# facebookresearch/momentum

Measured on NVIDIA H100. Metric: GN iterations/sec (batched 72-joint IK), higher is better.
Workload: dtype f32

## Files before the change

include/momentum_b200.h:

```cpp
#ifndef MOMENTUM_B200_H_
#define MOMENTUM_B200_H_

#include <stddef.h>
#include <stdint.h>

#ifdef __cplusplus
extern "C" {
#endif

#define MB2_PARAMETERS_PER_JOINT 7
#define MB2_MAX_MODEL_PARAMETERS 2048
#define MB2_PARAMETER_SET_WORDS 32

typedef enum mb2_status {
  MB2_OK = 0,
  MB2_ERR_INVALID_ARGUMENT = 1,
  MB2_ERR_CUDA = 2,
  MB2_ERR_UNSUPPORTED = 3
} mb2_status;

typedef enum mb2_instance_status {
  MB2_INSTANCE_OK = 0,
  MB2_INSTANCE_CHOLESKY_BREAKDOWN = 1,
  MB2_INSTANCE_NON_FINITE = 2
// ... 152 lines not shown
int mb2_solver_create(mb2_solver_function* f, const mb2_gauss_newton_options* opt, mb2_solver** out);
void mb2_solver_destroy(mb2_solver* s);
int mb2_solver_set_options(mb2_solver* s, const mb2_gauss_newton_options* opt);
int mb2_solver_set_enabled_parameters(mb2_solver* s, const uint64_t bits[MB2_PARAMETER_SET_WORDS]);
int mb2_solver_solve(mb2_solver* s, float* parameters, double* errors, int32_t* iterations, int32_t* status);
int mb2_solver_solve_async(mb2_solver* s, float* parameters);
int mb2_solver_wait(mb2_solver* s, double* errors, int32_t* iterations, int32_t* status);
int mb2_solver_solve_device(mb2_solver* s, float* parameters_device, void* cuda_stream);
int mb2_solver_get_results(mb2_solver* s, double* errors, int32_t* iterations, int32_t* status);
int mb2_solver_get_error_history(mb2_solver* s, double* history);
int mb2_solver_get_counters(mb2_solver* s, uint64_t* total_iterations, uint64_t* kernel_launches);
int mb2_solver_set_profiling(mb2_solver* s, int32_t enabled);
int mb2_solver_get_phase_times(mb2_solver* s, double ms[4], uint64_t launches[4]);
int mb2_solver_get_plan_stats(mb2_solver* s, int64_t stats[12]);
int mb2_solver_get_fused_profile(mb2_solver* s, int32_t* fused, int32_t* groups, double* kernel_ms, uint64_t phase_cycles[12]);
int mb2_solver_function_get_sweep_launch(mb2_solver_function* f, int32_t jacobian, int64_t out[5]);
int mb2_solver_get_solve_path(mb2_solver* s, int64_t out[15]);

typedef struct mb2_mixed_batch mb2_mixed_batch;
const char* mb2_mixed_batch_last_error(void);
int mb2_mixed_batch_create(int device, int32_t granule , mb2_mixed_batch** out);
void mb2_mixed_batch_destroy(mb2_mixed_batch* b);
int mb2_mixed_batch_add_rig(mb2_mixed_batch* b, const mb2_character* c, int32_t num_parameters, int32_t* rig_id);
int mb2_mixed_batch_use_limits(mb2_mixed_batch* b, int32_t enabled, float weight);
int mb2_mixed_batch_add_instance(mb2_mixed_batch* b, int32_t rig_id, int32_t num_constraints, const int32_t* parents, const float* offsets ,
                                 const float* weights , const float* targets , const float* theta0 , int32_t* instance_id);
int mb2_mixed_batch_set_parameters(mb2_mixed_batch* b, int32_t instance_id, const float* theta0);
int mb2_mixed_batch_solve(mb2_mixed_batch* b, const mb2_gauss_newton_options* opt);
int mb2_mixed_batch_get_result(mb2_mixed_batch* b, int32_t instance_id, float* theta, double* error, int32_t* iterations, int32_t* status);
int mb2_mixed_batch_get_results(mb2_mixed_batch* b, float* theta, const int64_t* theta_offsets, double* errors, int32_t* iterations, int32_t* status);
// ... 27 lines not shown
```

momentum_b200/csrc/ik_capi.cu:

```cuda
#include "../../include/momentum_b200.h"

#include <cuda_runtime.h>
#include <nvtx3/nvToolsExt.h>

#include <algorithm>
#include <cfloat>
#include <cmath>
#include <cstdio>
#include <cstdlib>
#include <cstring>
#include <memory>
#include <string>
#include <vector>

#include "ik_chol_sched.h"
#include "ik_fused.cuh"
#include "ik_jtj_tc.cuh"
#include "ik_kernels.cuh"
#include "ik_plan.h"
#include "ik_solve_path.h"

using namespace mb2;

namespace {
// ... 105 lines not shown
  const mb2_character* ch{nullptr};
  int B{0};
  cudaStream_t stream{nullptr};
  HostFunction host;
  bool planDirty{true};
  int planMode{0};
  bool planSchedDense{false};
  bool planAlignRows{false};
  uint64_t planLimitsVersion{~0ull};
  Plan plan;
  int ldJ{32};
  DeviceBuffer<EfDesc> dEfs;
  DeviceBuffer<UnitDesc> dUnits;
  DeviceBuffer<CellDesc> dCells;
  DeviceBuffer<ContribDesc> dContribs;
  DeviceBuffer<float> dLimitData;
  DeviceBuffer<int32_t> dEnabledList, dIdentity, dDeviceCols;
  DeviceBuffer<float> dTargets, dWeights, dJ, dTheta, dState, dH, dTargetStage;
  DeviceBuffer<double> dErrors;
  DeviceBuffer<double> dJacobi;
  std::unique_ptr<DeviceSchedule> sched;
  SweepLaunch lastSweep[2]{};
  FunctionTables tables() const;
};

struct PhaseEvent {
  cudaEvent_t start, stop;
  int phase;
};

struct mb2_solver {
  mb2_solver_function* fn{nullptr};
  mb2_gauss_newton_options opt{};
  DeviceBuffer<float> dH, dDelta, dThetaOrig, dTheta0, dScale, dGradDotDelta, dThetaStage, dGrad, dTiles, dRadius, dRSaved;
  DeviceBuffer<double> dLastErrors, dTrialErrors, dHistory;
  DeviceBuffer<int32_t> dActive, dIterations, dStatus, dSearching, dActiveCount, dWorkCounter, dQrChunks;
  DeviceBuffer<unsigned long long> dPhaseCycles;
  DeviceBuffer<float> dPark;
  DeviceBuffer<uint32_t> dParkSlots;
  SolvePath path;
  cudaEvent_t fusedStart{nullptr}, fusedStop{nullptr};
  double fusedMs{0};
  int* hActiveCount{nullptr};
  char* hResults{nullptr};
  size_t hResultsBytes{0};
  bool resultsStaged{false};
  uint64_t totalIterations{0}, kernelLaunches{0};
  bool profiling{false};
  bool inKernelProfile{false};
  std::vector<PhaseEvent> events;
  double phaseMs[4]{0, 0, 0, 0};
  uint64_t phaseLaunches[4]{0, 0, 0, 0};
// ... 36 lines not shown
  T.contribs = dContribs.p;
  T.limitData = dLimitData.p;
  T.targetStride = host.targetStride;
  T.recStride = plan.recStride;
  T.numRows = plan.numRows;
  T.ldJ = ldJ;
  T.numCols = plan.numCols;
  T.weightsPerInstance = host.weightsPerInstance ? 1 : 0;
  T.numWeights = host.numWeights;
  T.numContribs = int(plan.contribs.size());
  T.numLimitData = int(plan.limitData.size());
  const bool strips = planMode == 2 && planAlignRows && sched;
  T.stripMode = strips ? 1 : 0;
  T.residOff = strips ? sched->gram.residOff : 0;
  T.jacobianStride = strips ? size_t(sched->gram.stride) : size_t(plan.numCols + 1) * ldJ;
  return T;
}

namespace {

bool g_deviceChecked = false;
int g_usableDevices = 0;
}
namespace {
int usableDevices() {
  if (!g_deviceChecked) {
    int n = 0;
    if (cudaGetDeviceCount(&n) != cudaSuccess) { n = 0; cudaGetLastError(); }
    int ok = 0;
    for (int d = 0; d < n; ++d) {
// ... 72 lines not shown
        std::copy(ds->gc.tab.begin(), ds->gc.tab.end(), ds->gcParams->tab);
      } else if (ds->gcValid) {
        MB2_CUDA(ds->gcTab.upload(ds->gc.tab, s));
      }
      MB2_CUDA(ds->fBlob.upload(makeFusedBlob(f->ch->host, f->plan, gblob, sblob, ds->fLayout), s));
    }
    f->sched = std::move(ds);
  }
  f->planMode = mode;
  f->planSchedDense = schedDense;
  f->planAlignRows = alignRows;
  MB2_CUDA(f->dEfs.upload(f->plan.efs, s));
  MB2_CUDA(f->dUnits.upload(f->plan.units, s));
  MB2_CUDA(f->dCells.upload(f->plan.cells, s));
  MB2_CUDA(f->dContribs.upload(f->plan.contribs, s));
  MB2_CUDA(f->dLimitData.upload(f->plan.limitData, s));
  MB2_CUDA(f->dEnabledList.upload(f->plan.enabledList, s));
  MB2_CUDA(f->dDeviceCols.upload(f->plan.deviceCols, s));
  std::vector<int32_t> ident(f->ch->host.numParams);
  for (size_t i = 0; i < ident.size(); ++i) ident[i] = int32_t(i);
  MB2_CUDA(f->dIdentity.upload(ident, s));
  f->ldJ = std::max(32, roundUp(f->plan.numRows, 32));
  const bool stripLayout = mode == 2 && alignRows;
  const size_t jElems = stripLayout ? size_t(f->B) * size_t(f->sched->gram.stride) : size_t(f->B) * (f->plan.numCols + 1) * f->ldJ;
  MB2_CUDA(f->dJ.resize(jElems));
  MB2_CUDA(cudaMemsetAsync(f->dJ.p, 0, jElems * sizeof(float), s));
  MB2_CUDA(f->dErrors.resize(f->B));
  MB2_CUDA(f->dTheta.resize(size_t(f->B) * f->ch->host.numParams));
  int rc = ensureTargets(f);
  if (rc != MB2_OK) return rc;
// ... 846 lines not shown
  MB2_CUDA(s->dDelta.resize(size_t(B) * ns));
  MB2_CUDA(s->dTheta0.resize(size_t(B) * n));
  MB2_CUDA(s->dLastErrors.resize(B));
  MB2_CUDA(s->dActive.resize(B));
  MB2_CUDA(s->dActiveCount.resize(1));
  const bool lineSearch = o.do_line_search != 0 && P.kind != kSolveTrustRegionQr;
  if (lineSearch) {
    MB2_CUDA(s->dThetaOrig.resize(size_t(B) * n));
    MB2_CUDA(s->dTrialErrors.resize(B));
    MB2_CUDA(s->dScale.resize(B));
    MB2_CUDA(s->dSearching.resize(B));
    MB2_CUDA(s->dGradDotDelta.resize(B));
  }
  double* history = o.store_error_history ? s->dHistory.p : nullptr;

  const SweepArgs sweep = sweepArgs(f, theta, s->dActive.p);
  GramArgs g{};
  if (P.strips) {
    const DeviceSchedule& ds = *f->sched;
    g.batch = B;
    g.strips = f->dJ.p;
    g.stripStride = size_t(ds.gram.stride);
    g.residOff = ds.gram.residOff;
    g.active = s->dActive.p;
    g.numStrips = ds.gram.numStrips;
    g.numTiles = ds.host.numTiles;
    g.numTileCols = ds.host.numTileCols;
    g.nPad = ds.host.nPad;
    g.numOrder = int32_t(ds.gram.tileOrder.size());
    g.blob = ds.gBlob.p;
    g.blobInts = ds.gBlobInts;
// ... 287 lines not shown
    if ((persistent || gramChol) && s->profiling && s->dPhaseCycles.p) {
      MB2_DEVICE_GUARD(s->fn->ch->device);
      unsigned long long h[12];
      MB2_CUDA(cudaMemcpy(h, s->dPhaseCycles.p, sizeof(h), cudaMemcpyDeviceToHost));
      if (persistent) {
        for (int k = 0; k < 12; ++k) phaseCycles[k] = h[k];
      } else {
        phaseCycles[0] = h[0];
        for (int k = 1; k < 8; ++k) phaseCycles[4 + k] = h[k];
      }
    }
  }
  return MB2_OK;
}

int mb2_solver_function_get_sweep_launch(mb2_solver_function* f, int32_t jacobian, int64_t out[5]) {
  MB2_CHECK(f != nullptr && out != nullptr, "null argument");
  const SweepLaunch& l = f->lastSweep[jacobian ? 1 : 0];
  out[0] = l.stageTables;
  out[1] = l.warpsPerInstance;
  out[2] = l.groupsPerCta;
  out[3] = l.grid;
  out[4] = l.smemBytes;
  return MB2_OK;
}

int mb2_solver_get_solve_path(mb2_solver* s, int64_t out[15]) {
  MB2_CHECK(s != nullptr && out != nullptr, "null argument");
  solvePathWords(s->path, out);
  return MB2_OK;
// ... 13 lines not shown
```

momentum_b200/csrc/ik_device.cuh:

```cuda
#pragma once

#include <cmath>
#include <cfloat>

#include "ik_types.h"

namespace mb2 {

struct F3 {
  float x, y, z;
};
struct Q4 {
  float x, y, z, w;
};

MB2_HD F3 f3(float x, float y, float z) { F3 r; r.x = x; r.y = y; r.z = z; return r; }
MB2_HD F3 operator+(F3 a, F3 b) { return f3(a.x + b.x, a.y + b.y, a.z + b.z); }
MB2_HD F3 operator-(F3 a, F3 b) { return f3(a.x - b.x, a.y - b.y, a.z - b.z); }
MB2_HD F3 operator*(F3 a, float s) { return f3(a.x * s, a.y * s, a.z * s); }
MB2_HD F3 operator*(float s, F3 a) { return f3(a.x * s, a.y * s, a.z * s); }
MB2_HD float dot(F3 a, F3 b) { return a.x * b.x + a.y * b.y + a.z * b.z; }
MB2_HD F3 cross(F3 a, F3 b) { return f3(a.y * b.z - a.z * b.y, a.z * b.x - a.x * b.z, a.x * b.y - a.y * b.x); }
MB2_HD float comp(F3 a, int i) { return i == 0 ? a.x : (i == 1 ? a.y : a.z); }

// ... 260 lines not shown
#endif
  }
};
template <int kThreads>
struct CtaLanes {
  static constexpr int size = kThreads;
  int lane;
  MB2_HD void sync() const {
#if defined(__CUDA_ARCH__)
    __syncthreads();
#endif
  }
};
#endif

template <bool kAxes, bool kFromJointParameters, class Lanes>
MB2_HD void fkPasses(const Lanes& g, const CharacterTables& C, const float* src, float* js) {
  for (int j = g.lane; j < C.numJoints; j += g.size) {
    if constexpr (kFromJointParameters) fkLocal<kAxes>(C, j, src, js);
    else fkLocalFromTheta<kAxes>(C, j, src, js);
  }
  g.sync();
  for (int lvl = 1; lvl < C.numLevels; ++lvl) {
    const int end = C.levelStart[lvl + 1];
    for (int k = C.levelStart[lvl] + g.lane; k < end; k += g.size) fkCompose(C, C.levelJoints[k], js);
    g.sync();
  }
  if constexpr (kAxes)
    for (int i = g.lane; i < 3 * C.numJoints; i += g.size) fkAxis(C, i / 3, i % 3, js);
}

template <class Lanes>
MB2_HD void skelGradPasses(const Lanes& g, const CharacterTables& C, const SkeletonTables& S, const float* js, const float* grad, float* acc,
                           float* gjp, float* out) {
  for (int i = g.lane; i < C.numJoints; i += g.size) skelGradSeed(js, i, grad + 8 * i, acc);
  g.sync();
  for (int lvl = C.numLevels - 2; lvl >= 0; --lvl) {
    const int end = C.levelStart[lvl + 1];
    for (int k = C.levelStart[lvl] + g.lane; k < end; k += g.size) skelGradFold(S, js, C.levelJoints[k], acc);
    g.sync();
  }
  for (int row = g.lane; row < C.numJoints * kParametersPerJoint; row += g.size) gjp[row] = skelGradJointParameter(C, js, acc, row);
// ... 463 lines not shown
            }
          }
        }
      }
      const int nr = lm ? 6 : 12;
      for (int k = 0; k < nr; ++k) out[MB2_ROW(k)] = acc[k];
      break;
    }
    default:
      out[MB2_ROW(0)] = rc[0] * c.coef;
      break;
  }
#undef MB2_ROW
}

MB2_HD void skinTransform(const float* state, const float* ibp, float* m) {
  const Q4 q = qnormalized(ld4(state + 3));
  const float s = state[7];
  float R[9];
  qmat(q, R);
  for (int r = 0; r < 3; ++r) {
    const F3 sr = f3(s * R[r], s * R[3 + r], s * R[6 + r]);
    m[4 * r + 0] = dot(sr, f3(ibp[0], ibp[4], ibp[8]));
    m[4 * r + 1] = dot(sr, f3(ibp[1], ibp[5], ibp[9]));
    m[4 * r + 2] = dot(sr, f3(ibp[2], ibp[6], ibp[10]));
    m[4 * r + 3] = dot(sr, f3(ibp[3], ibp[7], ibp[11])) + state[r];
  }
}
MB2_HD F3 skinBlend(const SkinTables& S, const float* M, int v, F3 x) {
  F3 p = f3(0.f, 0.f, 0.f);
// ... 52 lines not shown
```

momentum_b200/csrc/ik_kernels.cu:

```cuda
#include "ik_kernels.cuh"

#include <algorithm>
#include <cstdio>
#include <type_traits>

#include "ik_chol.cuh"
#include "ik_chol_sched.h"
#include "ik_jtj_tc.cuh"
#include "ik_ptx.cuh"
#include "ik_device.cuh"
#include "ik_jacobi.cuh"

namespace mb2 {

__device__ __forceinline__ double warpSum(double v) {
  for (int o = 16; o > 0; o >>= 1) v += __shfl_xor_sync(0xffffffffu, v, o);
  return v;
}

size_t sweepSmemPerInstance(const FunctionTables& T, int warpsPerInstance) {
  const size_t nPad = (T.numParams + 3) & ~3;
  const size_t jp = warpsPerInstance > 1 ? size_t((T.numJoints * kParametersPerJoint + 1) & ~1) : 0;
  return sizeof(float) * (nPad + jp + size_t((T.numJoints * kJointStateStride + 1) & ~1) + size_t((T.recStride + 1) & ~1) + 4 + 2 * size_t(warpsPerInstance));
}

MB2_HD size_t tableWords(size_t count, size_t elemBytes) { return (count * elemBytes + 15) / 16 * 4; }
size_t characterTableWords(const CharacterTables& C) {
  const size_t J = C.numJoints;
  size_t w = tableWords(J, 4) + tableWords(3 * J, 4) + tableWords(4 * J, 4);
  w += tableWords(7 * J + 1, 4) + tableWords(C.ptNnz, 4) * 2 + tableWords(7 * J, 4);
  w += tableWords(C.numLevels + 1, 4) + tableWords(J, 4);
  return w;
}
size_t sweepTableBytes(const FunctionTables& T, int mode) {
  if (mode == 0) return 0;
  size_t w = characterTableWords(T);
  w += tableWords(T.numEf, sizeof(EfDesc)) + tableWords(T.numUnits, sizeof(UnitDesc)) + tableWords(T.numLimitData, 4);
  if (mode == 1) w += tableWords(T.numCells, sizeof(CellDesc)) + tableWords(T.numContribs, sizeof(ContribDesc));
  return w * 4;
}

template <class E>
__device__ __forceinline__ void stageTable(const E*& table, size_t count, uint32_t*& cursor) {
  static_assert(sizeof(E) % 4 == 0, "tables are staged word by word");
  const uint32_t* src = reinterpret_cast<const uint32_t*>(table);
  const size_t words = count * (sizeof(E) / 4);
  const int nt = int(blockDim.x);
  size_t i = threadIdx.x;
  for (; i + 7 * size_t(nt) < words; i += 8 * size_t(nt)) {
    uint32_t v[8];
#pragma unroll
    for (int k = 0; k < 8; ++k) v[k] = src[i + size_t(k) * nt];
#pragma unroll
    for (int k = 0; k < 8; ++k) cursor[i + size_t(k) * nt] = v[k];
  }
  for (; i < words; i += nt) cursor[i] = src[i];
  table = reinterpret_cast<const E*>(cursor);
  cursor += tableWords(count, sizeof(E));
}
__device__ __forceinline__ void stageCharacterTables(CharacterTables& C, uint32_t*& cursor) {
  const size_t J = C.numJoints;
  stageTable(C.parent, J, cursor); stageTable(C.offset, 3 * J, cursor); stageTable(C.prerot, 4 * J, cursor);
  stageTable(C.ptOuter, 7 * J + 1, cursor); stageTable(C.ptInner, C.ptNnz, cursor); stageTable(C.ptVals, C.ptNnz, cursor);
  stageTable(C.ptOffsets, 7 * J, cursor);
  stageTable(C.levelStart, C.numLevels + 1, cursor); stageTable(C.levelJoints, J, cursor);
}

constexpr int kSweepMaxWarps = 24;
template <bool kJacobian, int W, int kStage>
__global__ void __launch_bounds__(32 * kSweepMaxWarps) sweepKernel(const SweepArgs a) {
  extern __shared__ __align__(16) float smem[];
  FunctionTables T = a.T;
  const int warp = threadIdx.x >> 5, lane = threadIdx.x & 31;
  const WarpLanes<W> g = WarpLanes<W>::of(warp, lane);
  const int groupsPerCta = (blockDim.x >> 5) / W;
  const int nPad = (T.numParams + 3) & ~3;
  const int jpFloats = W > 1 ? ((T.numJoints * kParametersPerJoint + 1) & ~1) : 0;
  const int perGroup = nPad + jpFloats + ((T.numJoints * kJointStateStride + 1) & ~1) + ((T.recStride + 1) & ~1) + 4 + 2 * W;
  float* th = smem + size_t(g.group) * perGroup;
  float* jp = W > 1 ? th + nPad : nullptr;
  float* js = th + nPad + jpFloats;
  float* rec = js + ((T.numJoints * kJointStateStride + 1) & ~1);
  double* errSlots = reinterpret_cast<double*>(rec + ((T.recStride + 1) & ~1));
  if constexpr (kStage != 0) {
    uint32_t* cursor = reinterpret_cast<uint32_t*>(smem + ((size_t(groupsPerCta) * perGroup + 3) & ~size_t(3)));
    stageCharacterTables(T, cursor);
    stageTable(T.efs, T.numEf, cursor); stageTable(T.units, T.numUnits, cursor); stageTable(T.limitData, T.numLimitData, cursor);
    if constexpr (kStage == 1) { stageTable(T.cells, T.numCells, cursor); stageTable(T.contribs, T.numContribs, cursor); }
    __syncthreads();
  }

  for (int b = blockIdx.x * groupsPerCta + g.group; b < a.batch; b += gridDim.x * groupsPerCta) {
    if (a.active != nullptr && a.active[b] == 0) continue;
    const float* theta = a.theta + size_t(b) * a.ldTheta;
    for (int i = g.lane; i < T.numParams; i += g.size) th[i] = theta[i];
    g.sync();
    if (W == 1) {
      const int bn = b + gridDim.x * groupsPerCta;
      if (bn < a.batch) { const float* tn = a.theta + size_t(bn) * a.ldTheta; for (int i = g.lane * 8; i < T.numParams; i += g.size * 8) asm volatile("prefetch.global.L2 [%0];" ::"l"(tn + i)); }
    }
    if constexpr (W > 1) {
      for (int row = g.lane; row < T.numJoints * kParametersPerJoint; row += g.size) jp[row] = jointParameterRow(T, row, th);
      g.sync();
    }
    fkPasses<kJacobian, (W > 1)>(g, T, W > 1 ? jp : th, js);
    if constexpr (kJacobian) g.sync();
    if (a.stateOut != nullptr) {
      float* so = a.stateOut + size_t(b) * T.numJoints * 8;
      for (int i = g.lane; i < T.numJoints * 8; i += g.size) so[i] = js[(i >> 3) * kJointStateStride + (i & 7)];
    }
    const float* targets = a.targets + size_t(b) * T.targetStride;
    const float* cw = a.cweights + (T.weightsPerInstance ? size_t(b) * T.numWeights : 0);
    float* J = kJacobian ? a.jacobian + size_t(b) * T.jacobianStride : nullptr;
    float* residual = kJacobian ? J + (T.stripMode ? size_t(T.residOff) : size_t(T.numCols) * T.ldJ) : nullptr;
    double err = 0.0;
    for (int u = g.lane; u < T.numUnits; u += g.size) err += (double)evalUnit<kJacobian>(T, u, th, jp, js, targets, cw, rec, residual);
    err = warpSum(err);
    if (W > 1 && lane == 0) errSlots[warp % W] = err;
    g.sync();
    if (kJacobian)
      for (int c = g.lane; c < T.numCells; c += g.size) jacobianCell(T, c, js, rec, targets, J);
    if (g.lane == 0) {
      if (W > 1) { err = 0.0; for (int w = 0; w < W; ++w) err += errSlots[w]; }
      a.errors[b] = kJacobian ? err : (double)(float)err;
    }
    g.sync();
  }
}

static int g_numSms = 0;
static int g_maxSmemOptin = 0;
static int g_maxSmemPerSm = 0;

cudaError_t launchSweep(const SweepArgs& a0, bool jacobian, cudaStream_t stream, SweepLaunch* out) {
  SweepArgs a = a0;
  if (out) *out = SweepLaunch{};
  const size_t budget = size_t(g_maxSmemOptin);
  const size_t per1 = sweepSmemPerInstance(a.T, 8);
  a.stageTables = (2 * per1 + sweepTableBytes(a.T, 1) + 16 <= budget) ? 1 : (2 * per1 + sweepTableBytes(a.T, 2) + 16 <= budget) ? 2 : 0;
  const size_t tableBytes = sweepTableBytes(a.T, a.stageTables) + 16;
  int groups = int((budget - tableBytes) / per1);
  if (groups < 1) return cudaErrorInvalidConfiguration;
// ... 1 lines not shown
  int W = 1;
  if (groupsOneWarp >= 16) {
    const int sms = std::max(g_numSms, 1);
    const int maxG = std::min(groupsOneWarp, kSweepMaxWarps), minG = std::min(12, maxG);
    long best = -1;
    if (a.batch < sms * minG) { groups = std::max(1, (a.batch + sms - 1) / sms); best = 0; }
    for (int gcand = maxG; gcand >= minG && best != 0; --gcand) {
      const long rounds = (a.batch + long(sms) * gcand - 1) / (long(sms) * gcand);
      if (best < 0 || rounds * gcand < best) { best = rounds * gcand; groups = gcand; }
    }
  } else {
    if (groups > 15) groups = 15;
    while (W < 8 && groups * W * 2 <= kSweepMaxWarps) W *= 2;
  }
  a.warpsPerInstance = W;
  const int warps = groups * W;
  const size_t per = sweepSmemPerInstance(a.T, W);
  const size_t smem = per * groups + tableBytes;
  if (smem > budget) return cudaErrorInvalidConfiguration;
  const int ctasNeeded = (a.batch + groups - 1) / groups;
  int ctasPerSm = (int)((size_t(g_maxSmemPerSm)) / (smem + 1024));
  if (ctasPerSm < 1) ctasPerSm = 1;
  if (ctasPerSm * warps > 32) ctasPerSm = 32 / warps > 0 ? 32 / warps : 1;
  int grid = g_numSms * ctasPerSm;
  if (grid > ctasNeeded) grid = ctasNeeded;
  if (grid < 1) grid = 1;
  if (out) *out = SweepLaunch{a.stageTables, W, groups, grid, int64_t(smem)};
  auto launch = [&](auto kernel) -> cudaError_t {
    const cudaError_t e = cudaFuncSetAttribute(kernel, cudaFuncAttributeMaxDynamicSharedMemorySize, int(smem));
    if (e != cudaSuccess) return e;
    kernel<<<grid, warps * 32, smem, stream>>>(a);
    return cudaGetLastError();
  };
  auto pick = [&](auto jac, auto staged) -> cudaError_t {
    constexpr bool kJ = decltype(jac)::value;
    constexpr int kS = decltype(staged)::value;
    switch (W) {
      case 1: return launch(sweepKernel<kJ, 1, kS>);
      case 2: return launch(sweepKernel<kJ, 2, kS>);
      case 4: return launch(sweepKernel<kJ, 4, kS>);
      default: return launch(sweepKernel<kJ, 8, kS>);
    }
  };
  auto pickStage = [&](auto jac) -> cudaError_t {
    switch (a.stageTables) {
      case 1: return pick(jac, std::integral_constant<int, 1>{});
      case 2: return pick(jac, std::integral_constant<int, 2>{});
      default: return pick(jac, std::integral_constant<int, 0>{});
    }
  };
  return jacobian ? pickStage(std::true_type{}) : pickStage(std::false_type{});
// ... 1154 lines not shown
```

momentum_b200/csrc/ik_kernels.cuh:

```cuda
#pragma once

#include <cuda_runtime.h>

#include "ik_chol_sched.cuh"
#include "ik_chol_sched.h"
#include "ik_solve_path.h"
#include "ik_types.h"

namespace mb2 {

struct SweepArgs {
  FunctionTables T;
  int32_t batch;
  const float* theta;
  int32_t ldTheta;
  const float* targets;
  const float* cweights;
  float* jacobian;
  double* errors;
  const int32_t* active;
  float* stateOut;
  int32_t stageTables;
  int32_t warpsPerInstance;
};

struct JtJArgs {
  int32_t batch;
  const float* jacobian;
  int32_t numCols, ldJ, kRows;
  int32_t ns;
  float* H;
  int32_t ldH;
  size_t hStride;
  const int32_t* active;
  float* g;
  int32_t ldG;
};

// ... 196 lines not shown
```

momentum_b200/csrc/ik_plan.cpp:

```cpp
#include "ik_plan.h"

#include <algorithm>
#include <cfloat>
#include <cmath>
#include <cstring>
#include <map>

namespace mb2 {

std::string HostCharacter::validate() const {
  const int J = numJoints;
  if (J <= 0) return "skeleton has no joints";
  if (numParams <= 0 || numParams > 2048) return "number of model parameters must be in [1, 2048] (ParameterSet is bitset<2048>)";
  if (int(parent.size()) != J || int(offset.size()) != 3 * J || int(prerot.size()) != 4 * J) return "joint array sizes do not match the joint count";
  for (int j = 0; j < J; ++j)
    if (parent[j] >= j || parent[j] < -1) return "skeleton is not topologically sorted: parent index must precede child (skeleton.h:23-24)";
  const int rows = J * kParametersPerJoint;
  if (int(ptOuter.size()) != rows + 1 || int(ptOffsets.size()) != rows) return "parameter transform must have 7 * numJoints rows";
  if (ptOuter[0] != 0) return "parameter transform outer index must start at 0";
  for (int r = 0; r < rows; ++r)
    if (ptOuter[r + 1] < ptOuter[r]) return "parameter transform outer index must be non-decreasing";
  if (ptOuter[rows] != int(ptInner.size()) || ptInner.size() != ptVals.size()) return "parameter transform nnz mismatch";
  for (int c : ptInner)
    if (c < 0 || c >= numParams) return "parameter transform column out of range";
// ... 700 lines not shown
  std::vector<std::vector<int>> cliques(plan.units.size());
  for (const CellDesc& c : plan.cells) cliques[c.unit].push_back(int(c.col));
  const std::vector<int> prio = columnDepthPriority(ch, plan.enabledList);
  err = buildCholSchedule(plan.numCols, cliques, densePattern, sched, &prio);
  if (!err.empty()) return err;
  std::vector<int32_t> colOrder;
  layoutDeviceColumns(sched, colOrder);
  for (int32_t& c : colOrder) if (c >= 0) c = plan.enabledList[c];
  err = buildPlan(ch, efs, enabled, true, plan, &colOrder, strips);
  if (!err.empty() || !strips) return err;
  std::vector<int32_t> cr0, crn, cc;
  for (const CellDesc& c : plan.cells) { cr0.push_back(plan.units[c.unit].row0); crn.push_back(plan.units[c.unit].numRows); cc.push_back(int32_t(c.col)); }
  err = buildGramPlan(sched, cr0, crn, cc, plan.numRows, gram);
  if (!err.empty()) return err;
  for (size_t i = 0; i < plan.cells.size(); ++i) { plan.cells[i].stripOff = gram.cellStripOff[i]; plan.cells[i].quadStride = gram.cellQuadStride[i]; }
  return "";
}

}
```

momentum_b200/csrc/ik_plan.h:

```cpp
#pragma once

#include <cstdint>
#include <string>
#include <vector>

#include "../../include/momentum_b200.h"
#include "ik_chol_sched.h"
#include "ik_types.h"

namespace mb2 {

struct HostLimit {
  int32_t type;
  float weight;
  int32_t i[4];
  float f[27];
};

struct HostCharacter {
  int32_t numJoints{0}, numParams{0};
  std::vector<int32_t> parent;
  std::vector<float> offset, prerot;
  std::vector<int32_t> ptOuter, ptInner;
  std::vector<float> ptVals, ptOffsets;
// ... 74 lines not shown
std::string limitErrorFunction(float weight, float alpha, float c, HostErrorFunction& out);

struct Plan {
  std::vector<EfDesc> efs;
  std::vector<UnitDesc> units;
  std::vector<CellDesc> cells;
  std::vector<ContribDesc> contribs;
  std::vector<float> limitData;
  int32_t numRows{0};
  int32_t recStride{0};
  int32_t actualParameters{0};
  std::vector<int32_t> enabledList;
  int32_t numCols{0};
  bool compact{false};
  std::vector<int32_t> deviceCols;
};

std::string buildPlan(const HostCharacter& ch, const std::vector<HostErrorFunction>& efs, const std::vector<uint8_t>& enabled, bool compact, Plan& out,
                      const std::vector<int32_t>* columnOrder = nullptr, bool alignRowGroups = false);

int32_t jacobianBlockSize(const HostCharacter& ch, const HostErrorFunction& ef);

int resolveCholeskyMode(int requested, const std::vector<uint8_t>& enabled);

std::string planSolverPath(const HostCharacter& ch, const std::vector<HostErrorFunction>& efs, const std::vector<uint8_t>& enabled, bool densePattern, bool strips,
                           Plan& plan, CholSchedule& sched, GramPlan& gram);

}
```

momentum_b200/csrc/ik_types.h:

```cpp
#pragma once

#include <cstdint>

#if defined(__CUDACC__)
#define MB2_HD __host__ __device__ __forceinline__
#else
#define MB2_HD inline
#endif

namespace mb2 {

constexpr int kParametersPerJoint = 7;
constexpr int kJointStateStride = 17;
constexpr float kLn2 = 0.69314718055994530942f;
constexpr float kPi = 3.14159265358979323846f;

enum UnitKind : int32_t {
  kUnitPosition = 0,
  kUnitOrientation = 1,
  kUnitOrientationRotDiff = 2,
  kUnitStateMatrix = 3,
  kUnitStateLogMap = 4,
  kUnitLimitMinMax = 5,
  kUnitLimitMinMaxJoint = 6,
// ... 36 lines not shown
  uint16_t unit;
  uint16_t col;
  uint32_t contribBegin;
  uint16_t contribCount;
  uint16_t quadStride;
  float coef;
  uint32_t stripOff;
};

struct ContribDesc {
  uint16_t joint;
  uint16_t dof;
  float coef;
};

struct CharacterTables {
  int32_t numJoints, numParams;
  const int32_t* parent;
  const float* offset;
  const float* prerot;
  const int32_t* ptOuter;
  const int32_t* ptInner;
  const float* ptVals;
  const float* ptOffsets;
  int32_t numLevels;
  const int32_t* levelStart;
  const int32_t* levelJoints;
  int32_t ptNnz;
};

// ... 2 lines not shown
  const EfDesc* efs;
  const UnitDesc* units;
  const CellDesc* cells;
  const ContribDesc* contribs;
  const float* limitData;
  int32_t targetStride;
  int32_t recStride;
  int32_t numRows;
  int32_t ldJ;
  int32_t numCols;
  int32_t weightsPerInstance;
  int32_t numWeights;
  int32_t numContribs, numLimitData;
  int32_t stripMode, residOff;
  size_t jacobianStride;
};

struct SkeletonTables {
  const int32_t* childStart;
  const int32_t* children;
  const int32_t* ptColStart;
  const int32_t* ptColRows;
  const float* ptColVals;
};

constexpr int kSkinMaxInfluences = 8;
constexpr int kSkinSegment = 128;
constexpr int kSkinIbpStride = 12;
struct SkinTables {
  int32_t numVertices, numSegments;
// ... 14 lines not shown
```

momentum_b200/solver.py:

```python
from __future__ import annotations

import ctypes as C
import os
from dataclasses import dataclass
from typing import List, Optional, Sequence

import numpy as np

from . import character as mc

_HERE = os.path.dirname(os.path.abspath(__file__))
DEFAULT_LIB = os.path.join(_HERE, "lib", "libmomentum_b200.so")

SIZE_MAX = 2 ** 64 - 1

JTJ_AUTO, JTJ_FP32_SIMT, JTJ_TF32X3, JTJ_TF32, JTJ_SPARSE_TILES = 0, 1, 2, 3, 4
INSTANCE_OK, INSTANCE_CHOLESKY_BREAKDOWN, INSTANCE_NON_FINITE = 0, 1, 2
CHOLESKY_AUTO, CHOLESKY_DENSE_EIGEN, CHOLESKY_TILES_DENSE, CHOLESKY_TILES_SPARSE = 0, 1, 2, 3
FUSED_AUTO, FUSED_OFF, FUSED_PERSISTENT, FUSED_GRAM_CHOLESKY = 0, 1, 2, 3
FUSED_ON = FUSED_PERSISTENT
LINEAR_SOLVER_CHOLESKY, LINEAR_SOLVER_QR, LINEAR_SOLVER_TRUST_REGION_QR = 0, 1, 2


class MomentumB200Error(RuntimeError):
# ... 16 lines not shown
_ip = C.POINTER(C.c_int32)
_dp = C.POINTER(C.c_double)
_up = C.POINTER(C.c_uint64)

CABI_SYMBOLS = [
    "mb2_last_error", "mb2_device_count", "mb2_default_gauss_newton_options", "mb2_character_create", "mb2_character_set_parameter_limits",
    "mb2_character_destroy", "mb2_solver_function_create", "mb2_solver_function_destroy", "mb2_solver_function_num_parameters",
    "mb2_solver_function_actual_parameters", "mb2_solver_function_batch", "mb2_solver_function_jacobian_rows",
    "mb2_solver_function_jacobian_stride", "mb2_add_position_error_function", "mb2_add_position_error_function_instanced", "mb2_add_orientation_error_function",
    "mb2_add_plane_error_function", "mb2_add_model_parameters_error_function",
    "mb2_add_state_error_function", "mb2_add_limit_error_function", "mb2_set_error_function_weight", "mb2_set_targets",
    "mb2_set_targets_device", "mb2_set_constraint_weights", "mb2_solver_function_set_enabled_parameters", "mb2_solver_function_get_error",
    "mb2_solver_function_get_jacobian", "mb2_solver_function_get_jtjr", "mb2_solver_function_get_skeleton_state", "mb2_solver_create",
    "mb2_solver_destroy", "mb2_solver_set_options", "mb2_solver_set_enabled_parameters", "mb2_solver_solve", "mb2_solver_solve_device",
    "mb2_solver_get_results", "mb2_solver_get_error_history", "mb2_solver_get_counters", "mb2_solver_set_profiling",
    "mb2_solver_get_phase_times", "mb2_solver_get_plan_stats", "mb2_solver_get_fused_profile", "mb2_solver_solve_async", "mb2_solver_wait",
    "mb2_set_constraint_weights_device", "mb2_solver_function_get_jacobian_device",
    "mb2_mixed_batch_last_error", "mb2_mixed_batch_create", "mb2_mixed_batch_destroy", "mb2_mixed_batch_add_rig", "mb2_mixed_batch_use_limits",
    "mb2_mixed_batch_add_instance", "mb2_mixed_batch_set_parameters", "mb2_mixed_batch_solve", "mb2_mixed_batch_get_result", "mb2_mixed_batch_get_results",
    "mb2_mixed_batch_stats", "mb2_mixed_batch_bucket_info",
    "mb2_character_clone", "mb2_solver_function_clone", "mb2_character_device", "mb2_solver_function_character", "mb2_solver_function_num_error_functions",
    "mb2_solver_function_target_size", "mb2_sharded_last_error", "mb2_sharded_solver_create", "mb2_sharded_solver_destroy", "mb2_sharded_solver_num_shards",
    "mb2_sharded_solver_shard_info", "mb2_sharded_solver_set_options", "mb2_sharded_solver_set_targets", "mb2_sharded_solver_solve", "mb2_sharded_solver_get_aggregate",
    "mb2_character_skeleton_state_device", "mb2_character_skeleton_state_backward_device",
    "mb2_add_orientation_error_function_instanced", "mb2_solver_function_input_gradients_device",
    "mb2_solver_function_implicit_direction_device", "mb2_solver_function_get_sweep_launch", "mb2_solver_get_solve_path",
    "mb2_character_set_skinning", "mb2_character_num_vertices", "mb2_character_skin_points_device", "mb2_character_skin_points_backward_device",
]

_libs = {}

# ... 38 lines not shown
    L.mb2_solver_destroy.argtypes = [vp]
    L.mb2_solver_set_options.argtypes = [vp, C.POINTER(_Options)]
    L.mb2_solver_set_enabled_parameters.argtypes = [vp, _up]
    L.mb2_solver_solve.argtypes = [vp, vp, _dp, _ip, _ip]
    if hasattr(L, "mb2_solver_solve_device"):
        L.mb2_solver_solve_device.argtypes = [vp, vp, vp]
        L.mb2_solver_get_results.argtypes = [vp, _dp, _ip, _ip]
        L.mb2_solver_set_profiling.argtypes = [vp, C.c_int32]
        L.mb2_solver_get_phase_times.argtypes = [vp, _dp, _up]
    L.mb2_solver_get_error_history.argtypes = [vp, _dp]
    L.mb2_solver_get_counters.argtypes = [vp, _up, _up]
    if hasattr(L, "mb2_solver_get_plan_stats"):
        L.mb2_solver_get_plan_stats.argtypes = [vp, C.POINTER(C.c_int64)]
    if hasattr(L, "mb2_solver_get_fused_profile"):
        L.mb2_solver_get_fused_profile.argtypes = [vp, _ip, _ip, _dp, _up]
    L.mb2_default_gauss_newton_options.argtypes = [C.POINTER(_Options)]
    if hasattr(L, "mb2_set_constraint_weights_device"):
        L.mb2_set_constraint_weights_device.argtypes = [vp, C.c_int32, vp, vp]
        L.mb2_solver_function_get_jacobian_device.argtypes = [vp, vp, C.POINTER(vp), _ip, vp]
    if hasattr(L, "mb2_mixed_batch_create"):
        L.mb2_solver_solve_async.argtypes = [vp, vp]
        L.mb2_solver_wait.argtypes = [vp, _dp, _ip, _ip]
        L.mb2_mixed_batch_last_error.restype = C.c_char_p
        L.mb2_mixed_batch_create.argtypes = [C.c_int, C.c_int32, C.POINTER(vp)]
        L.mb2_mixed_batch_destroy.argtypes = [vp]
        L.mb2_mixed_batch_add_rig.argtypes = [vp, vp, C.c_int32, _ip]
        L.mb2_mixed_batch_use_limits.argtypes = [vp, C.c_int32, C.c_float]
        L.mb2_mixed_batch_add_instance.argtypes = [vp, C.c_int32, C.c_int32, _ip, _fp, _fp, _fp, _fp, _ip]
        L.mb2_mixed_batch_set_parameters.argtypes = [vp, C.c_int32, _fp]
        L.mb2_mixed_batch_solve.argtypes = [vp, C.POINTER(_Options)]
# ... 388 lines not shown
    def get_plan_stats(self):
        st = (C.c_int64 * 12)()
        self._check(self._L.mb2_solver_get_plan_stats(self._h, st))
        keys = ["jacobian_nonzeros", "jacobian_columns", "ldj", "normal_parameters", "cholesky_tiles", "cholesky_tile_ops", "cholesky_levels", "rows",
                "strip_floats", "gram_macs", "gram_pairs", "fused_groups"]
        return dict(zip(keys, (int(v) for v in st)))

    FUSED_PHASES = ["fetch", "joint_parameters", "fk", "units", "cells", "gram", "parked_tiles", "chol_diag", "chol_panel", "chol_update",
                    "chol_backward", "update_bookkeeping"]

    def get_fused_profile(self):
        fused = C.c_int32(0); groups = C.c_int32(0); ms_ = C.c_double(0.0); cyc = (C.c_uint64 * 12)()
        self._check(self._L.mb2_solver_get_fused_profile(self._h, C.byref(fused), C.byref(groups), C.byref(ms_), cyc))
        return {"fused": int(fused.value), "groups": groups.value, "kernel_ms": ms_.value, "phase_cycles": dict(zip(self.FUSED_PHASES, (int(v) for v in cyc)))}

    SOLVE_PATH_KINDS = {0: None, 1: "dense", 2: "tiles_kmajor", 3: "tiles", 4: "gram_cholesky", 5: "persistent", 6: "qr", 7: "trust_region_qr"}
    SOLVE_PATH_KEYS = ["kind", "plan_mode", "sched_dense", "strips", "jtj_mode", "dense_nb", "dense_in_smem", "gram_threads", "chol_threads",
                       "qr_max_chunk_rows", "qr_chunks", "qr_widest_chunk", "tr_r_floats", "fused_groups", "fused_smem"]

    def get_solve_path(self) -> dict:
        out = (C.c_int64 * 15)()
        self._check(self._L.mb2_solver_get_solve_path(self._h, out))
        d = dict(zip(self.SOLVE_PATH_KEYS, (int(v) for v in out)))
        d["kind"] = self.SOLVE_PATH_KINDS[d["kind"]]
        return d

    def set_profiling(self, level):
        self._check(self._L.mb2_solver_set_profiling(self._h, int(level)))

    def get_phase_times(self):
# ... 128 lines not shown
```

Before: 9.610 million.

## Precompile Jacobian cells into segmented 16-byte stream records for the sweep kernel

Adds a host-built cell stream that groups Jacobian cells by kind (single-contribution point, multi-contribution point, orientation) into packed 16-byte records with precomputed joint-state slots. The sweep kernel gains a stage-3 path that stages these tables in shared memory and evaluates each segment with a specialised branch-free loop and vector stores, falling back to the generic per-cell path for the rest. The aim is to cut per-cell descriptor decoding, branching and divergence in the Jacobian fill. It also adds optional in-kernel clock profiling of sweep phases. The cost is extra shared memory for the new tables and an extra kernel specialisation.

```diff
diff --git a/include/momentum_b200.h b/include/momentum_b200.h
--- a/include/momentum_b200.h
+++ b/include/momentum_b200.h
@@ -190,6 +190,7 @@
 int mb2_solver_get_phase_times(mb2_solver* s, double ms[4], uint64_t launches[4]);
 int mb2_solver_get_plan_stats(mb2_solver* s, int64_t stats[12]);
 int mb2_solver_get_fused_profile(mb2_solver* s, int32_t* fused, int32_t* groups, double* kernel_ms, uint64_t phase_cycles[12]);
+int mb2_solver_get_sweep_profile(mb2_solver* s, uint64_t phase_cycles[8]);
 int mb2_solver_function_get_sweep_launch(mb2_solver_function* f, int32_t jacobian, int64_t out[5]);
 int mb2_solver_get_solve_path(mb2_solver* s, int64_t out[15]);
 
diff --git a/momentum_b200/csrc/ik_capi.cu b/momentum_b200/csrc/ik_capi.cu
--- a/momentum_b200/csrc/ik_capi.cu
+++ b/momentum_b200/csrc/ik_capi.cu
@@ -143,6 +143,10 @@
   DeviceBuffer<UnitDesc> dUnits;
   DeviceBuffer<CellDesc> dCells;
   DeviceBuffer<ContribDesc> dContribs;
+  DeviceBuffer<CellRecord> dStream;
+  DeviceBuffer<StreamContrib> dStreamContribs;
+  DeviceBuffer<CellDesc> dStreamCells;
+  DeviceBuffer<ContribDesc> dStreamCellContribs;
   DeviceBuffer<float> dLimitData;
   DeviceBuffer<int32_t> dEnabledList, dIdentity, dDeviceCols;
   DeviceBuffer<float> dTargets, dWeights, dJ, dTheta, dState, dH, dTargetStage;
@@ -165,6 +169,7 @@
   DeviceBuffer<double> dLastErrors, dTrialErrors, dHistory;
   DeviceBuffer<int32_t> dActive, dIterations, dStatus, dSearching, dActiveCount, dWorkCounter, dQrChunks;
   DeviceBuffer<unsigned long long> dPhaseCycles;
+  DeviceBuffer<unsigned long long> dSweepCycles;
   DeviceBuffer<float> dPark;
   DeviceBuffer<uint32_t> dParkSlots;
   SolvePath path;
@@ -231,6 +236,16 @@
   T.stripMode = strips ? 1 : 0;
   T.residOff = strips ? sched->gram.residOff : 0;
   T.jacobianStride = strips ? size_t(sched->gram.stride) : size_t(plan.numCols + 1) * ldJ;
+  if (strips) {
+    for (int k = 0; k <= kStreamSegments; ++k) T.streamSeg[k] = plan.streamSeg[k];
+    T.numStreamContribs = int(plan.streamContribs.size());
+    T.numStreamCells = int(plan.streamCells.size());
+    T.numStreamCellContribs = int(plan.streamCellContribs.size());
+    T.stream = dStream.p;
+    T.streamContribs = dStreamContribs.p;
+    T.streamCells = dStreamCells.p;
+    T.streamCellContribs = dStreamCellContribs.p;
+  }
   return T;
 }
 
@@ -333,6 +348,10 @@
   MB2_CUDA(f->dUnits.upload(f->plan.units, s));
   MB2_CUDA(f->dCells.upload(f->plan.cells, s));
   MB2_CUDA(f->dContribs.upload(f->plan.contribs, s));
+  MB2_CUDA(f->dStream.upload(f->plan.stream, s));
+  MB2_CUDA(f->dStreamContribs.upload(f->plan.streamContribs, s));
+  MB2_CUDA(f->dStreamCells.upload(f->plan.streamCells, s));
+  MB2_CUDA(f->dStreamCellContribs.upload(f->plan.streamCellContribs, s));
   MB2_CUDA(f->dLimitData.upload(f->plan.limitData, s));
   MB2_CUDA(f->dEnabledList.upload(f->plan.enabledList, s));
   MB2_CUDA(f->dDeviceCols.upload(f->plan.deviceCols, s));
@@ -1209,7 +1228,12 @@
   }
   double* history = o.store_error_history ? s->dHistory.p : nullptr;
 
-  const SweepArgs sweep = sweepArgs(f, theta, s->dActive.p);
+  SweepArgs sweep = sweepArgs(f, theta, s->dActive.p);
+  if (s->inKernelProfile) {
+    MB2_CUDA(s->dSweepCycles.resize(kSweepProfileWords));
+    MB2_CUDA(cudaMemsetAsync(s->dSweepCycles.p, 0, kSweepProfileWords * sizeof(unsigned long long), st));
+    sweep.phaseCycles = s->dSweepCycles.p;
+  }
   GramArgs g{};
   if (P.strips) {
     const DeviceSchedule& ds = *f->sched;
@@ -1527,6 +1551,18 @@
   return MB2_OK;
 }
 
+int mb2_solver_get_sweep_profile(mb2_solver* s, uint64_t phaseCycles[8]) {
+  MB2_CHECK(s != nullptr && phaseCycles != nullptr, "null argument");
+  for (int k = 0; k < kSweepProfileWords; ++k) phaseCycles[k] = 0;
+  if (s->profiling && s->inKernelProfile && s->dSweepCycles.p) {
+    MB2_DEVICE_GUARD(s->fn->ch->device);
+    unsigned long long h[kSweepProfileWords];
+    MB2_CUDA(cudaMemcpy(h, s->dSweepCycles.p, sizeof(h), cudaMemcpyDeviceToHost));
+    for (int k = 0; k < kSweepProfileWords; ++k) phaseCycles[k] = h[k];
+  }
+  return MB2_OK;
+}
+
 int mb2_solver_function_get_sweep_launch(mb2_solver_function* f, int32_t jacobian, int64_t out[5]) {
   MB2_CHECK(f != nullptr && out != nullptr, "null argument");
   const SweepLaunch& l = f->lastSweep[jacobian ? 1 : 0];
diff --git a/momentum_b200/csrc/ik_device.cuh b/momentum_b200/csrc/ik_device.cuh
--- a/momentum_b200/csrc/ik_device.cuh
+++ b/momentum_b200/csrc/ik_device.cuh
@@ -298,18 +298,23 @@
 };
 #endif
 
-template <bool kAxes, bool kFromJointParameters, class Lanes>
-MB2_HD void fkPasses(const Lanes& g, const CharacterTables& C, const float* src, float* js) {
+struct NoPassMark {
+  MB2_HD void operator()(int) const {}
+};
+template <bool kAxes, bool kFromJointParameters, class Lanes, class Mark = NoPassMark>
+MB2_HD void fkPasses(const Lanes& g, const CharacterTables& C, const float* src, float* js, Mark mark = Mark{}) {
   for (int j = g.lane; j < C.numJoints; j += g.size) {
     if constexpr (kFromJointParameters) fkLocal<kAxes>(C, j, src, js);
     else fkLocalFromTheta<kAxes>(C, j, src, js);
   }
   g.sync();
+  mark(0);
   for (int lvl = 1; lvl < C.numLevels; ++lvl) {
     const int end = C.levelStart[lvl + 1];
     for (int k = C.levelStart[lvl] + g.lane; k < end; k += g.size) fkCompose(C, C.levelJoints[k], js);
     g.sync();
   }
+  mark(1);
   if constexpr (kAxes)
     for (int i = g.lane; i < 3 * C.numJoints; i += g.size) fkAxis(C, i / 3, i % 3, js);
 }
@@ -803,6 +808,77 @@
 #undef MB2_ROW
 }
 
+MB2_HD F3 slotDerivative(const float* js, uint32_t slot, F3 v) {
+  const float* p = js + (slot & 0xffffu);
+  const int d = int(slot >> 16) & 7;
+  if (d < 3) {
+    if (slot & kSlotRootTranslation) return f3(d == 0 ? 1.f : 0.f, d == 1 ? 1.f : 0.f, d == 2 ? 1.f : 0.f);
+    return qmatcol(ld4(p + 3), d) * p[7];
+  }
+  const F3 off = v - ld3(p);
+  if (d < 6) return cross(ld3(p + 8 + 3 * (d - 3)), off);
+  return off * kLn2;
+}
+MB2_HD void storePointCell(float* out, F3 acc) {
+#if defined(__CUDA_ARCH__)
+  *reinterpret_cast<float4*>(out) = make_float4(acc.x, acc.y, acc.z, 0.f);
+#else
+  out[0] = acc.x; out[1] = acc.y; out[2] = acc.z;
+#endif
+}
+
+template <class Lanes>
+MB2_HD void jacobianStream(const Lanes& g, const FunctionTables& T, const float* js, const float* rec, const float* targets, float* J) {
+  for (int i = T.streamSeg[kStreamPointSingle] + g.lane; i < T.streamSeg[kStreamPointSingle + 1]; i += g.size) {
+    const CellRecord c = T.stream[i];
+    const float* rc = rec + c.recOff;
+    const F3 v = ld3(rc);
+    const float ds = rc[3];
+    F3 acc = f3(0.f, 0.f, 0.f);
+    acc = acc + (slotDerivative(js, c.slot, v) * ds) * c.coef;
+    storePointCell(J + c.stripOff, acc);
+  }
+  for (int i = T.streamSeg[kStreamPointMulti] + g.lane; i < T.streamSeg[kStreamPointMulti + 1]; i += g.size) {
+    const CellRecord c = T.stream[i];
+    const float* rc = rec + c.recOff;
+    const F3 v = ld3(rc);
+    const float ds = rc[3];
+    const StreamContrib* cb = T.streamContribs + c.slot;
+    F3 acc = f3(0.f, 0.f, 0.f);
+    for (int k = 0; k < c.run.count; ++k) acc = acc + (slotDerivative(js, cb[k].slot, v) * ds) * cb[k].coef;
+    storePointCell(J + c.stripOff, acc);
+  }
+  for (int i = T.streamSeg[kStreamOrientation] + g.lane; i < T.streamSeg[kStreamOrientation + 1]; i += g.size) {
+    const CellRecord c = T.stream[i];
+    const float* rc = rec + c.recOff;
+    const float ds = rc[9];
+    const StreamContrib* cb = T.streamContribs + c.slot;
+    float acc[9];
+    for (int k = 0; k < 9; ++k) acc[k] = 0.f;
+    for (int k = 0; k < c.run.count; ++k) {
+      const uint32_t s = cb[k].slot;
+      const F3 axis = ld3(js + (s & 0xffffu) + 8 + 3 * ((int(s >> 16) & 7) - 3));
+      for (int jv = 0; jv < 3; ++jv) {
+        const F3 d = cross(axis, ld3(rc + 3 * jv));
+        acc[3 * jv] += (ds * d.x) * cb[k].coef; acc[3 * jv + 1] += (ds * d.y) * cb[k].coef; acc[3 * jv + 2] += (ds * d.z) * cb[k].coef;
+      }
+    }
+    float* out = J + c.stripOff;
+    const int quadFloats = int(c.run.quadStride) * 64;
+#if defined(__CUDA_ARCH__)
+    *reinterpret_cast<float4*>(out) = make_float4(acc[0], acc[1], acc[2], acc[3]);
+    *reinterpret_cast<float4*>(out + quadFloats) = make_float4(acc[4], acc[5], acc[6], acc[7]);
+    *reinterpret_cast<float4*>(out + 2 * quadFloats) = make_float4(acc[8], 0.f, 0.f, 0.f);
+#else
+    for (int k = 0; k < 9; ++k) out[(k >> 2) * quadFloats + (k & 3)] = acc[k];
+#endif
+  }
+  FunctionTables R = T;
+  R.cells = T.streamCells;
+  R.contribs = T.streamCellContribs;
+  for (int i = g.lane; i < T.numStreamCells; i += g.size) jacobianCell(R, i, js, rec, targets, J);
+}
+
 MB2_HD void skinTransform(const float* state, const float* ibp, float* m) {
   const Q4 q = qnormalized(ld4(state + 3));
   const float s = state[7];
diff --git a/momentum_b200/csrc/ik_kernels.cu b/momentum_b200/csrc/ik_kernels.cu
--- a/momentum_b200/csrc/ik_kernels.cu
+++ b/momentum_b200/csrc/ik_kernels.cu
@@ -37,6 +37,9 @@
   size_t w = characterTableWords(T);
   w += tableWords(T.numEf, sizeof(EfDesc)) + tableWords(T.numUnits, sizeof(UnitDesc)) + tableWords(T.numLimitData, 4);
   if (mode == 1) w += tableWords(T.numCells, sizeof(CellDesc)) + tableWords(T.numContribs, sizeof(ContribDesc));
+  if (mode == 3)
+    w += tableWords(T.streamSeg[kStreamSegments], sizeof(CellRecord)) + tableWords(T.numStreamContribs, sizeof(StreamContrib)) +
+         tableWords(T.numStreamCells, sizeof(CellDesc)) + tableWords(T.numStreamCellContribs, sizeof(ContribDesc));
   return w * 4;
 }
 
@@ -67,7 +70,8 @@
 }
 
 constexpr int kSweepMaxWarps = 24;
-template <bool kJacobian, int W, int kStage>
+enum SweepPhase { kSweepTheta, kSweepFkLocal, kSweepFkCompose, kSweepAxes, kSweepUnits, kSweepCells, kSweepErrorWrite, kSweepPhases };
+template <bool kJacobian, int W, int kStage, bool kProfile = false>
 __global__ void __launch_bounds__(32 * kSweepMaxWarps) sweepKernel(const SweepArgs a) {
   extern __shared__ __align__(16) float smem[];
   FunctionTables T = a.T;
@@ -87,11 +91,24 @@
     stageCharacterTables(T, cursor);
     stageTable(T.efs, T.numEf, cursor); stageTable(T.units, T.numUnits, cursor); stageTable(T.limitData, T.numLimitData, cursor);
     if constexpr (kStage == 1) { stageTable(T.cells, T.numCells, cursor); stageTable(T.contribs, T.numContribs, cursor); }
-    __syncthreads();
-  }
+    if constexpr (kStage == 3) {
+      stageTable(T.stream, size_t(T.streamSeg[kStreamSegments]), cursor); stageTable(T.streamContribs, T.numStreamContribs, cursor);
+      stageTable(T.streamCells, T.numStreamCells, cursor); stageTable(T.streamCellContribs, T.numStreamCellContribs, cursor);
+    }
+    __syncthreads();
+  }
+  const bool profiler = kProfile && blockIdx.x == gridDim.x / 2 && warp == 0 && lane == 0;
+  unsigned pc[kSweepPhases + 1] = {};
+  unsigned pt = 0;
+  auto mark = [&](int phase) {
+    if constexpr (kProfile) {
+      if (profiler) { const unsigned now = unsigned(clock()); pc[phase] += now - pt; pt = now; }
+    }
+  };
 
   for (int b = blockIdx.x * groupsPerCta + g.group; b < a.batch; b += gridDim.x * groupsPerCta) {
     if (a.active != nullptr && a.active[b] == 0) continue;
+    if constexpr (kProfile) { pt = unsigned(clock()); pc[kSweepPhases] += 1; }
     const float* theta = a.theta + size_t(b) * a.ldTheta;
     for (int i = g.lane; i < T.numParams; i += g.size) th[i] = theta[i];
     g.sync();
@@ -103,8 +120,10 @@
       for (int row = g.lane; row < T.numJoints * kParametersPerJoint; row += g.size) jp[row] = jointParameterRow(T, row, th);
       g.sync();
     }
-    fkPasses<kJacobian, (W > 1)>(g, T, W > 1 ? jp : th, js);
+    mark(kSweepTheta);
+    fkPasses<kJacobian, (W > 1)>(g, T, W > 1 ? jp : th, js, [&](int pass) { mark(pass == 0 ? kSweepFkLocal : kSweepFkCompose); });
     if constexpr (kJacobian) g.sync();
+    mark(kSweepAxes);
     if (a.stateOut != nullptr) {
       float* so = a.stateOut + size_t(b) * T.numJoints * 8;
       for (int i = g.lane; i < T.numJoints * 8; i += g.size) so[i] = js[(i >> 3) * kJointStateStride + (i & 7)];
@@ -118,14 +137,24 @@
     err = warpSum(err);
     if (W > 1 && lane == 0) errSlots[warp % W] = err;
     g.sync();
-    if (kJacobian)
+    mark(kSweepUnits);
+    if constexpr (kJacobian && kStage == 3) {
+      jacobianStream(g, T, js, rec, targets, J);
+    } else if constexpr (kJacobian) {
       for (int c = g.lane; c < T.numCells; c += g.size) jacobianCell(T, c, js, rec, targets, J);
+    }
+    if constexpr (kProfile) __syncwarp();
+    mark(kSweepCells);
     if (g.lane == 0) {
       if (W > 1) { err = 0.0; for (int w = 0; w < W; ++w) err += errSlots[w]; }
       a.errors[b] = kJacobian ? err : (double)(float)err;
     }
     g.sync();
-  }
+    mark(kSweepErrorWrite);
+  }
+  if constexpr (kProfile)
+    if (profiler && a.phaseCycles != nullptr)
+      for (int k = 0; k <= kSweepPhases; ++k) a.phaseCycles[k] = pc[k];
 }
 
 static int g_numSms = 0;
@@ -157,9 +186,10 @@
     while (W < 8 && groups * W * 2 <= kSweepMaxWarps) W *= 2;
   }
   a.warpsPerInstance = W;
+  const bool cellStream = jacobian && a.stageTables == 1 && W == 1 && a.T.stripMode && a.T.stream != nullptr;
   const int warps = groups * W;
   const size_t per = sweepSmemPerInstance(a.T, W);
-  const size_t smem = per * groups + tableBytes;
+  const size_t smem = per * groups + (cellStream ? sweepTableBytes(a.T, 3) + 16 : tableBytes);
   if (smem > budget) return cudaErrorInvalidConfiguration;
   const int ctasNeeded = (a.batch + groups - 1) / groups;
   int ctasPerSm = (int)((size_t(g_maxSmemPerSm)) / (smem + 1024));
@@ -175,9 +205,14 @@
     kernel<<<grid, warps * 32, smem, stream>>>(a);
     return cudaGetLastError();
   };
+  const bool profile = jacobian && W == 1 && a.phaseCycles != nullptr;
   auto pick = [&](auto jac, auto staged) -> cudaError_t {
     constexpr bool kJ = decltype(jac)::value;
     constexpr int kS = decltype(staged)::value;
+    if constexpr (kJ) {
+      if (cellStream) return profile ? launch(sweepKernel<true, 1, 3, true>) : launch(sweepKernel<true, 1, 3>);
+      if (profile) return launch(sweepKernel<true, 1, kS, true>);
+    }
     switch (W) {
       case 1: return launch(sweepKernel<kJ, 1, kS>);
       case 2: return launch(sweepKernel<kJ, 2, kS>);
diff --git a/momentum_b200/csrc/ik_kernels.cuh b/momentum_b200/csrc/ik_kernels.cuh
--- a/momentum_b200/csrc/ik_kernels.cuh
+++ b/momentum_b200/csrc/ik_kernels.cuh
@@ -9,6 +9,7 @@
 
 namespace mb2 {
 
+constexpr int kSweepProfileWords = 8;
 struct SweepArgs {
   FunctionTables T;
   int32_t batch;
@@ -22,6 +23,7 @@
   float* stateOut;
   int32_t stageTables;
   int32_t warpsPerInstance;
+  unsigned long long* phaseCycles;
 };
 
 struct JtJArgs {
diff --git a/momentum_b200/csrc/ik_plan.cpp b/momentum_b200/csrc/ik_plan.cpp
--- a/momentum_b200/csrc/ik_plan.cpp
+++ b/momentum_b200/csrc/ik_plan.cpp
@@ -738,7 +738,53 @@
   err = buildGramPlan(sched, cr0, crn, cc, plan.numRows, gram);
   if (!err.empty()) return err;
   for (size_t i = 0; i < plan.cells.size(); ++i) { plan.cells[i].stripOff = gram.cellStripOff[i]; plan.cells[i].quadStride = gram.cellQuadStride[i]; }
-  return "";
-}
-
-}
+  buildCellStream(ch, plan);
+  return "";
+}
+
+void buildCellStream(const HostCharacter& ch, Plan& plan) {
+  plan.stream.clear(); plan.streamContribs.clear(); plan.streamCells.clear(); plan.streamCellContribs.clear();
+  const bool slotsFit = size_t(ch.numJoints) * kJointStateStride <= 0xffffu;
+  auto slotOf = [&](const ContribDesc& k) -> uint32_t {
+    const int par = ch.parent[k.joint];
+    if (k.dof >= 3) return uint32_t(k.joint * kJointStateStride) | (uint32_t(k.dof) << 16);
+    if (par < 0) return kSlotRootTranslation | (uint32_t(k.dof) << 16);
+    return uint32_t(par * kJointStateStride) | (uint32_t(k.dof) << 16);
+  };
+  auto segmentOf = [&](const CellDesc& c) -> int {
+    const UnitDesc& u = plan.units[c.unit];
+    if (!slotsFit || (u.row0 & 3) != 0 || c.contribCount == 0) return kStreamSegments;
+    if (u.kind == kUnitPosition || u.kind == kUnitLimitEllipsoid) return c.contribCount == 1 ? kStreamPointSingle : kStreamPointMulti;
+    return u.kind == kUnitOrientation ? kStreamOrientation : kStreamSegments;
+  };
+  for (int s = 0; s <= kStreamSegments; ++s) {
+    plan.streamSeg[s] = int32_t(plan.stream.size());
+    if (s == kStreamSegments) break;
+    for (const CellDesc& c : plan.cells) {
+      if (segmentOf(c) != s) continue;
+      const ContribDesc* cb = plan.contribs.data() + c.contribBegin;
+      CellRecord r{};
+      r.stripOff = c.stripOff;
+      r.recOff = uint32_t(plan.units[c.unit].recOff);
+      if (s == kStreamPointSingle) {
+        r.slot = slotOf(cb[0]);
+        r.coef = cb[0].coef;
+      } else {
+        r.slot = uint32_t(plan.streamContribs.size());
+        r.run.count = c.contribCount;
+        r.run.quadStride = c.quadStride;
+        for (int k = 0; k < c.contribCount; ++k) plan.streamContribs.push_back(StreamContrib{slotOf(cb[k]), cb[k].coef});
+      }
+      plan.stream.push_back(r);
+    }
+  }
+  for (const CellDesc& c : plan.cells) {
+    if (segmentOf(c) != kStreamSegments) continue;
+    CellDesc d = c;
+    d.contribBegin = uint32_t(plan.streamCellContribs.size());
+    plan.streamCellContribs.insert(plan.streamCellContribs.end(), plan.contribs.begin() + c.contribBegin, plan.contribs.begin() + c.contribBegin + c.contribCount);
+    plan.streamCells.push_back(d);
+  }
+}
+
+}
diff --git a/momentum_b200/csrc/ik_plan.h b/momentum_b200/csrc/ik_plan.h
--- a/momentum_b200/csrc/ik_plan.h
+++ b/momentum_b200/csrc/ik_plan.h
@@ -112,7 +112,14 @@
   int32_t numCols{0};
   bool compact{false};
   std::vector<int32_t> deviceCols;
+  std::vector<CellRecord> stream;
+  int32_t streamSeg[kStreamSegments + 1]{};
+  std::vector<StreamContrib> streamContribs;
+  std::vector<CellDesc> streamCells;
+  std::vector<ContribDesc> streamCellContribs;
 };
+
+void buildCellStream(const HostCharacter& ch, Plan& plan);
 
 std::string buildPlan(const HostCharacter& ch, const std::vector<HostErrorFunction>& efs, const std::vector<uint8_t>& enabled, bool compact, Plan& out,
                       const std::vector<int32_t>* columnOrder = nullptr, bool alignRowGroups = false);
diff --git a/momentum_b200/csrc/ik_types.h b/momentum_b200/csrc/ik_types.h
--- a/momentum_b200/csrc/ik_types.h
+++ b/momentum_b200/csrc/ik_types.h
@@ -74,6 +74,23 @@
   float coef;
 };
 
+enum StreamSegment : int32_t { kStreamPointSingle = 0, kStreamPointMulti = 1, kStreamOrientation = 2, kStreamSegments = 3 };
+constexpr uint32_t kSlotRootTranslation = 1u << 19;
+struct StreamContrib {
+  uint32_t slot;
+  float coef;
+};
+struct CellRecord {
+  uint32_t stripOff;
+  uint32_t recOff;
+  uint32_t slot;
+  union {
+    float coef;
+    struct { uint16_t count, quadStride; } run;
+  };
+};
+static_assert(sizeof(CellRecord) == 16, "one 16-byte record per cell");
+
 struct CharacterTables {
   int32_t numJoints, numParams;
   const int32_t* parent;
@@ -106,6 +123,12 @@
   int32_t numContribs, numLimitData;
   int32_t stripMode, residOff;
   size_t jacobianStride;
+  int32_t streamSeg[kStreamSegments + 1];
+  int32_t numStreamContribs, numStreamCells, numStreamCellContribs;
+  const CellRecord* stream;
+  const StreamContrib* streamContribs;
+  const CellDesc* streamCells;
+  const ContribDesc* streamCellContribs;
 };
 
 struct SkeletonTables {
diff --git a/momentum_b200/solver.py b/momentum_b200/solver.py
--- a/momentum_b200/solver.py
+++ b/momentum_b200/solver.py
@@ -54,7 +54,7 @@
     "mb2_solver_function_get_jacobian", "mb2_solver_function_get_jtjr", "mb2_solver_function_get_skeleton_state", "mb2_solver_create",
     "mb2_solver_destroy", "mb2_solver_set_options", "mb2_solver_set_enabled_parameters", "mb2_solver_solve", "mb2_solver_solve_device",
     "mb2_solver_get_results", "mb2_solver_get_error_history", "mb2_solver_get_counters", "mb2_solver_set_profiling",
-    "mb2_solver_get_phase_times", "mb2_solver_get_plan_stats", "mb2_solver_get_fused_profile", "mb2_solver_solve_async", "mb2_solver_wait",
+    "mb2_solver_get_phase_times", "mb2_solver_get_plan_stats", "mb2_solver_get_fused_profile", "mb2_solver_get_sweep_profile", "mb2_solver_solve_async", "mb2_solver_wait",
     "mb2_set_constraint_weights_device", "mb2_solver_function_get_jacobian_device",
     "mb2_mixed_batch_last_error", "mb2_mixed_batch_create", "mb2_mixed_batch_destroy", "mb2_mixed_batch_add_rig", "mb2_mixed_batch_use_limits",
     "mb2_mixed_batch_add_instance", "mb2_mixed_batch_set_parameters", "mb2_mixed_batch_solve", "mb2_mixed_batch_get_result", "mb2_mixed_batch_get_results",
@@ -123,6 +123,8 @@
         L.mb2_solver_get_plan_stats.argtypes = [vp, C.POINTER(C.c_int64)]
     if hasattr(L, "mb2_solver_get_fused_profile"):
         L.mb2_solver_get_fused_profile.argtypes = [vp, _ip, _ip, _dp, _up]
+    if hasattr(L, "mb2_solver_get_sweep_profile"):
+        L.mb2_solver_get_sweep_profile.argtypes = [vp, _up]
     L.mb2_default_gauss_newton_options.argtypes = [C.POINTER(_Options)]
     if hasattr(L, "mb2_set_constraint_weights_device"):
         L.mb2_set_constraint_weights_device.argtypes = [vp, C.c_int32, vp, vp]
@@ -541,6 +543,13 @@
         self._check(self._L.mb2_solver_get_fused_profile(self._h, C.byref(fused), C.byref(groups), C.byref(ms_), cyc))
         return {"fused": int(fused.value), "groups": groups.value, "kernel_ms": ms_.value, "phase_cycles": dict(zip(self.FUSED_PHASES, (int(v) for v in cyc)))}
 
+    SWEEP_PHASES = ["theta_load", "fk_local", "fk_compose", "axes", "units", "cells", "error_write"]
+
+    def get_sweep_profile(self):
+        cyc = (C.c_uint64 * 8)()
+        self._check(self._L.mb2_solver_get_sweep_profile(self._h, cyc))
+        return {"instances": int(cyc[7]), "phase_cycles": dict(zip(self.SWEEP_PHASES, (int(v) for v in cyc[:7])))}
+
     SOLVE_PATH_KINDS = {0: None, 1: "dense", 2: "tiles_kmajor", 3: "tiles", 4: "gram_cholesky", 5: "persistent", 6: "qr", 7: "trust_region_qr"}
     SOLVE_PATH_KEYS = ["kind", "plan_mode", "sched_dense", "strips", "jtj_mode", "dense_nb", "dense_in_smem", "gram_threads", "chol_threads",
                        "qr_max_chunk_rows", "qr_chunks", "qr_widest_chunk", "tr_r_floats", "fused_groups", "fused_smem"]
```

After: 9.778 million, median of 6. 1.02x the previous value.
